# facebookresearch/FBTT-Embedding

Measured on AMD Instinct MI355X. Metric: fwd+bwd GFLOPS (true algorithmic: 3 x fwd FLOP / time), TT-EmbeddingBag E=11M D=64 ranks=[32, 32] nnz=10240, higher is better.
Workload: dtype f32

## Files before the change

### fbtt-embedding_amd/csrc/ttx_tt.hip

```cpp
#include "ttx_tt_common.h"

namespace ttx {

#include "ttx_tt_generic.inc"

__global__ __launch_bounds__(kThreads) void pool_kernel(int Nmax, const int* __restrict__ hdr, int B, int D,
                                                       const int64_t* __restrict__ rowidx,
                                                       const int64_t* __restrict__ tableidx,
                                                       const float* __restrict__ rows,
                                                       const float* __restrict__ psw, float* __restrict__ out) {
  const int n = blockIdx.x * (kThreads / 32) + threadIdx.x / 32;
  const int l = threadIdx.x & 31;
  const int N = min(Nmax, hdr[2]);
  if (n >= N) return;
  const int64_t r = rowidx[n], tb = tableidx[n];
  if (n > 0 && rowidx[n - 1] == r && tableidx[n - 1] == tb) return;
  const unsigned long long half = (threadIdx.x & 32) ? 0xffffffff00000000ull : 0x00000000ffffffffull;
  int sl = 1;
  for (;;) {
    const int c = n + sl + l;
    const bool same = c < N && rowidx[c] == r && tableidx[c] == tb;
    unsigned long long m = (__ballot(!same) & half) >> (threadIdx.x & 32);
    if (m) { sl += __builtin_ctzll(m); break; }
    sl += 32;
// ... 961 lines not shown
    return;
  }
  constexpr int kOwnerBlock = 256;
  for (int e = tid; e < sl; e += nthreads) {
    float g = 0.f;
    for (int i0 = beg; i0 < end; i0 += kOwnerBlock) {
      const int i1 = min(end, i0 + kOwnerBlock);
      float part = 0.f;
      for (int i = i0; i < i1; ++i) part += pc[(list ? (size_t)list[i] : (size_t)i) * sl + e];
      g += part;
    }
    if (optim == TTX_OPTIM_DENSE) {
      dw[base + e] = g;
    } else {
      float sv = optim == TTX_OPTIM_ADAGRAD ? stt[base + e] : 0.f;
      wt[base + e] = apply_one(optim, g, wt[base + e], lr, eps, &sv);
      if (optim == TTX_OPTIM_ADAGRAD) stt[base + e] = sv;
    }
  }
}

#include "ttx_tt_spec.inc"

static bool spec_shape(const Dims& d) { return spec_match(d) != SPEC_NONE; }
#ifndef TTX_SUBCHUNK_NNZ
#define TTX_SUBCHUNK_NNZ 131072
#endif
#ifndef TTX_SUBCHUNKS
#define TTX_SUBCHUNKS 4
#endif
template <class S>
constexpr int mc_of(int ks) { return S::MC * (S::SUB ? ks : 1); }
static int spec_mc(const Dims& d, long long nnz) {
  const int ks = nnz >= TTX_SUBCHUNK_NNZ ? TTX_SUBCHUNKS : 1;
  switch (spec_match(d)) {
    case SPEC_32_4_32_4: return mc_of<S_32_4_32_4>(ks);
    case SPEC_16_4_16_4: return mc_of<S_16_4_16_4>(ks);
    case SPEC_32_4_32_8: return mc_of<S_32_4_32_8>(ks);
    case SPEC_16_4_16_8: return mc_of<S_16_4_16_8>(ks);
    case SPEC_64_4_64_8: return mc_of<S_64_4_64_8>(ks);
    case SPEC_64_4_64_4: return mc_of<S_64_4_64_4>(ks);
    case SPEC2_32_4_32_4: return mc_of<S2_32_4_32_4>(ks);
    case SPEC2_16_4_16_4: return mc_of<S2_16_4_16_4>(ks);
    case SPEC2_64_4_64_4: return mc_of<S2_64_4_64_4>(ks);
    case SPEC_32_8_32_8: return mc_of<S_32_8_32_8>(ks);
    case SPEC_64_8_64_8: return mc_of<S_64_8_64_8>(ks);
    case SPEC2_32_2_32_4: return mc_of<S2_32_2_32_4>(ks);
    case SPEC2_64_2_64_4: return mc_of<S2_64_2_64_4>(ks);
    case SPEC2_16_2_16_4: return mc_of<S2_16_2_16_4>(ks);
    case SPEC_16_8_16_8: return mc_of<S_16_8_16_8>(ks);
    case SPEC_128_4_128_4: return mc_of<S_128_4_128_4>(ks);
    case SPEC_128_4_128_8: return mc_of<S_128_4_128_8>(ks);
    case SPEC_128_8_128_8: return mc_of<S_128_8_128_8>(ks);
    case SPEC_32_8_32_16: return mc_of<S_32_8_32_16>(ks);
    case SPEC_32_16_32_16: return mc_of<S_32_16_32_16>(ks);
    case SPEC_16_16_16_16: return mc_of<S_16_16_16_16>(ks);
    case SPEC_64_16_64_16: return mc_of<S_64_16_64_16>(ks);
    case SPEC_32_16_32_32: return mc_of<S_32_16_32_32>(ks);
    case SPEC_16_16_16_32: return mc_of<S_16_16_16_32>(ks);
    case SPEC_32_4_32_32: return mc_of<S_32_4_32_32>(ks);
    case SPEC_16_4_16_32: return mc_of<S_16_4_16_32>(ks);
    case SPEC_32_8_32_32: return mc_of<S_32_8_32_32>(ks);
    case SPEC_16_8_16_32: return mc_of<S_16_8_16_32>(ks);
    case SPEC_16_8_16_16: return mc_of<S_16_8_16_16>(ks);
    case SPEC_64_8_64_16: return mc_of<S_64_8_64_16>(ks);
    default: return 0;
  }
// ... 804 lines not shown
  TTX_HIP(hipGetLastError());
  return TTX_OK;
}

}

using namespace ttx;

extern "C" {

#ifdef TTX_TEST_HOOKS
int ttx_debug_stamps(void* device_buffer) {
  g_stamps = (long long*)device_buffer;
  return TTX_OK;
}

int ttx_debug_skip(int32_t mask) {
  g_disable_spec = (mask & 256) ? 1 : 0;
  g_disable_pad = (mask & 32768) ? 1 : 0;
  g_no_pack = (mask >> 16) & 1;
  g_skip_launch = (mask >> 9) & 63;
  mask &= 255;
  g_debug_skip = mask;
  return TTX_OK;
}

int ttx_debug_lds_budget(int32_t bytes) {
  if (bytes < 0 || bytes > 160 * 1024) TTX_FAIL(TTX_EINVAL, "LDS budget %d out of range", bytes);
  g_lds_budget = bytes ? bytes : 160 * 1024;
  return TTX_OK;
}

int ttx_set_chunk(int32_t mc) {
  if (mc < 0 || mc > 64) TTX_FAIL(TTX_EINVAL, "chunk %d out of range 0..64", mc);
  g_chunk_override = mc;
  return TTX_OK;
}
#endif

int ttx_debug_tiles(const ttx_geom* g, int32_t* out) {
  Dims d;
  int rc = make_dims(g, &d);
  if (rc) return rc;
  if (!out) TTX_FAIL(TTX_EINVAL, "out is NULL");
  for (int i = 0; i < 6; ++i) out[i] = 0;
  if (spec_shape(d) || t4_merge_dims(d, nullptr) || t2_shape(d)) return TTX_OK;
  const TileCfg cfg = choose_tiles(d);
  if (cfg.MC <= 0) return TTX_OK;
  const Lds L = make_lds(d, cfg.MC, true, cfg.bpp, cfg.KB);
  out[0] = L.MC; out[1] = L.bpp; out[2] = L.KB; out[3] = L.ncp; out[4] = L.nkb; out[5] = L.bytes;
  return TTX_OK;
}

int ttx_debug_state(void) {
  return ((g_debug_skip | g_skip_launch | g_disable_spec | g_disable_pad | g_no_pack) ? 1 : 0) | (g_lds_budget != 160 * 1024 ? 2 : 0) |
         (g_chunk_override ? 4 : 0) | (g_stamps ? 8 : 0) | (ttx_cache_debug_state() << 4);
}

int ttx_has_test_hooks(void) {
#ifdef TTX_TEST_HOOKS
  return 1;
#else
  return 0;
#endif
}

size_t ttx_tt_forward_workspace_bytes(const ttx_geom* g, int32_t B, int32_t D, int64_t nnz) {
// ... 628 lines not shown
```

### fbtt-embedding_amd/csrc/ttx_tt_common.h

```cpp
#pragma once
#include "ttx_internal.h"

namespace ttx {

constexpr int kThreads = 256;
constexpr int kWaves = kThreads / kWave;

typedef float f32x4 __attribute__((ext_vector_type(4)));

struct CorePtrs {
  float* c[TTX_MAX_CORES];
};

struct FastDiv {
  unsigned d;
  float rcp;
};
__host__ __device__ __forceinline__ FastDiv make_fd(int d) {
  FastDiv f;
  f.d = (unsigned)(d > 0 ? d : 1);
  f.rcp = 1.0f / (float)f.d;
  return f;
}
#define make_fd_dev make_fd
// ... 2 lines not shown
    rem = n % f.d;
    return n / f.d;
  }
  unsigned q = (unsigned)((float)n * f.rcp);
  int r = (int)n - (int)(q * f.d);
  if (r < 0) { q -= 1; r += (int)f.d; }
  else if (r >= (int)f.d) { q += 1; r -= (int)f.d; }
  rem = (unsigned)r;
  return q;
}

struct Partials {
  float* pc[TTX_MAX_CORES];
  const float* psw;
  const int64_t* tableidx;
  int* hot_cnt;
  int n_hot_cnt;
  float* seg[TTX_MAX_CORES];
};

__device__ __forceinline__ void zero_hot_counters(const Partials& PC) {
  if (blockIdx.x == 0 && PC.hot_cnt)
    for (int i = threadIdx.x; i < PC.n_hot_cnt; i += blockDim.x) PC.hot_cnt[i] = 0;
}

__device__ __forceinline__ f32x4 mfma4(float a, float b, f32x4 c) {
  return __builtin_amdgcn_mfma_f32_16x16x4f32(a, b, c, 0, 0, 0);
}

__device__ __forceinline__ f32x4 mfma1(float a, float b, f32x4 c) {
  return __builtin_amdgcn_mfma_f32_4x4x1f32(a, b, c, 0, 0, 0);
}

__device__ __forceinline__ void zero_output(float* __restrict__ out, long long n) {
  if (!out) return;
  for (long long e = (long long)blockIdx.x * kThreads + threadIdx.x; e < n; e += (long long)gridDim.x * kThreads) out[e] = 0.f;
}

#ifdef TTX_TEST_HOOKS
extern int g_debug_skip;
extern int g_disable_spec;
extern long long* g_stamps;
#else
constexpr int g_debug_skip = 0;
constexpr int g_disable_spec = 0;
constexpr long long* g_stamps = nullptr;
#endif

}
```

### fbtt-embedding_amd/csrc/ttx_tt_spec.inc

```

#ifndef TTX_SETPRIO
#define TTX_SETPRIO 0
#endif
#if TTX_SETPRIO
#define TTX_PRIO(x) __builtin_amdgcn_s_setprio(x)
#else
#define TTX_PRIO(x) do {} while (0)
#endif

#ifndef TTX_WGS32
#define TTX_WGS32 2
#endif
#ifndef TTX_MFMA_TAIL
#define TTX_MFMA_TAIL 1
#endif
#ifndef TTX_BFS
#define TTX_BFS 1
#endif
#ifndef TTX_GPP
#define TTX_GPP 1
#endif
#ifndef TTX_LATEB
#define TTX_LATEB 1
#endif
// ... 92 lines not shown
template <class S, bool PAD = false>
__device__ __forceinline__ void spec_fetch_b(const float* __restrict__ B1, int pass, BBlock<S>& b, const RealDims& R) {
  const int tid = threadIdx.x;
#pragma unroll
  for (int i = 0; i < S::BV4; ++i) {
    const int e = tid + i * kThreads;
    const int row = e / (S::BW / 4), c4 = e % (S::BW / 4);
    const int col0 = S::BFS ? 0 : pass * S::PW;
    if (S::BFULL || e < S::K0 * S::BW / 4) {
      if constexpr (!PAD) {
        b.v[i] = *(const float4*)(B1 + (size_t)row * S::N1 + col0 + c4 * 4);
      } else {
        const int col = col0 + c4 * 4;
        const int bq = col / S::R2, kk = col % S::R2;
        b.v[i] = ld4_guard(B1 + (size_t)row * R.n1 + bq * R.r2 + kk, (row < R.r1 && bq < R.q1) ? R.r2 - kk : 0, B1, (R.v4 & 2) != 0);
      }
    }
  }
}
template <class S>
__device__ __forceinline__ void spec_put_b(const BBlock<S>& b, float* Bs) {
  const int tid = threadIdx.x;
#pragma unroll
  for (int i = 0; i < S::BV4; ++i) {
    const int e = tid + i * kThreads;
    const int row = e / (S::BW / 4), c4 = e % (S::BW / 4);
    if (S::BFULL || e < S::K0 * S::BW / 4) {
      float2* dst = (float2*)(Bs + row * S::LDB + c4 * 4);
      dst[0] = make_float2(b.v[i].x, b.v[i].y);
      dst[1] = make_float2(b.v[i].z, b.v[i].w);
    }
  }
}
template <class S, bool ALLA>
__device__ __forceinline__ void spec_zero_pads(float* Bs, float* Aw) {
  const int tid = threadIdx.x, lane = lane_id();
  if (S::K0P != S::K0)
    for (int e = tid; e < (S::K0P - S::K0) * S::LDB; e += kThreads) Bs[S::K0 * S::LDB + e] = 0.f;
  if (ALLA || S::K0P != S::K0)
    for (int e = lane; e < S::RG * S::szA; e += kWave) Aw[e] = 0.f;
}

template <class S, bool TRANS = false>
__device__ __forceinline__ void spec_gemm_x0(const float* Aw, const float* Bs, f32x4 (&acc)[S::PNT]) {
  const int lane = lane_id();
  const int i16 = lane & 15, kq = lane >> 4;
  const float* arow = Aw + i16 * S::LDA + 8 * kq;
  const float* bbase = Bs + 8 * kq * S::LDB + i16;
#pragma unroll
  for (int x = 0; x < S::PNT; ++x) acc[x] = (f32x4){0.f, 0.f, 0.f, 0.f};
  float bcur[S::PNT];
#pragma unroll
  for (int x = 0; x < S::PNT; ++x) bcur[x] = bbase[x * 16];
  TTX_PRIO(1);
#pragma unroll
  for (int kb = 0; kb < S::K0P; kb += 32) {
    float a[8];
#pragma unroll
    for (int t = 0; t < 8; ++t) a[t] = arow[kb + t];
    __builtin_amdgcn_sched_group_barrier(0x100, 4, 0);
#pragma unroll
    for (int t = 0; t < 8; ++t) {
      const int kn = (t < 7) ? kb + t + 1 : kb + 32;
      const float* bn = bbase + (kn < S::K0P ? kn : 0) * S::LDB;
      float bnxt[S::PNT];
#pragma unroll
// ... 206 lines not shown
        if (live) L.av[gi][i] = *(const float4*)(C.c[0] + sid0 * S::SL0 + a * S::K0 + k);
      } else {
        L.av[gi][i] = ld4_guard(C.c[0] + sid0 * R.sl0 + a * R.r1 + k, (live && a < R.q0) ? R.r1 - k : 0, C.c[0], (R.v4 & 1) != 0);
      }
    }
#pragma unroll
    for (int hr = 0; hr < S::HH * 4; ++hr) {
      const int kk = (hr / 4) * 16 + kq * 4 + hr % 4;
      if constexpr (S::FMT) {
#pragma unroll
        for (int xb = 0; xb < S::Q2 / 4; ++xb) {
          const int x = 4 * xb + t4;
          if constexpr (!PAD) L.c2[gi][hr * (S::Q2 / 4) + xb] = C.c[2][sid2 * S::SL2 + kk * S::Q2 + x];
          else L.c2[gi][hr * (S::Q2 / 4) + xb] = ld_guard(C.c[2] + sid2 * R.sl2 + kk * R.q2 + x, kk < R.r2 && x < R.q2, C.c[2]);
        }
      } else if constexpr (!PAD) {
        const float4* cg = (const float4*)(C.c[2] + sid2 * S::SL2 + kk * S::Q2);
#pragma unroll
        for (int x4 = 0; x4 < S::Q2 / 4; ++x4) {
          const float4 t = cg[x4];
          L.c2[gi][hr * S::Q2 + 4 * x4] = t.x; L.c2[gi][hr * S::Q2 + 4 * x4 + 1] = t.y;
          L.c2[gi][hr * S::Q2 + 4 * x4 + 2] = t.z; L.c2[gi][hr * S::Q2 + 4 * x4 + 3] = t.w;
        }
      } else {
        const float* cg = C.c[2] + sid2 * R.sl2 + kk * R.q2;
#pragma unroll
        for (int x4 = 0; x4 < S::Q2 / 4; ++x4) {
          const float4 t = ld4_guard(cg + 4 * x4, kk < R.r2 ? R.q2 - 4 * x4 : 0, C.c[2], (R.v4 & 4) != 0);
          L.c2[gi][hr * S::Q2 + 4 * x4] = t.x; L.c2[gi][hr * S::Q2 + 4 * x4 + 1] = t.y;
          L.c2[gi][hr * S::Q2 + 4 * x4 + 2] = t.z; L.c2[gi][hr * S::Q2 + 4 * x4 + 3] = t.w;
        }
      }
    }
  }
}

#ifndef TTX_NO_KHEAD
#define TTX_KHEAD_PARAMS const int4* k_chunk_rec, const int4* k_lrec, const int* k_lrow, const int* k_hdr, const float* k_c0, \
                         const float* k_c1, const float* k_c2,
#define TTX_KHEAD_ARGS(P, C) (P).chunk_rec, (P).lrec, (P).lrow, (P).hdr, (C).c[0], (C).c[1], (C).c[2],
#define TTX_KHEAD_ADOPT(P, C)                                                                                         \
  do {                                                                                                                \
    (P).chunk_rec = const_cast<int4*>(k_chunk_rec); (P).lrec = const_cast<int4*>(k_lrec); (P).lrow = const_cast<int*>(k_lrow); \
    (P).hdr = const_cast<int*>(k_hdr); (C).c[0] = const_cast<float*>(k_c0); (C).c[1] = const_cast<float*>(k_c1);       \
    (C).c[2] = const_cast<float*>(k_c2);                                                                              \
  } while (0)
#else
#define TTX_KHEAD_PARAMS
#define TTX_KHEAD_ARGS(P, C)
#define TTX_KHEAD_ADOPT(P, C) do { } while (0)
#endif
template <class S, bool MULTI, bool FUSE = false, bool PAD = false>
__global__ __launch_bounds__(kThreads, S::WGS) void spec_fwd_kernel(TTX_KHEAD_PARAMS Plan P, CorePtrs C, float* __restrict__ rows,
                                                             float* __restrict__ zout, long long nzero, PoolFuse F, RealDims R) {
  extern __shared__ __attribute__((aligned(16))) float smem[];
  static_assert(!FUSE || (!MULTI && !PAD), "fused pooling: single sub-chunk, exact shape");
  TTX_KHEAD_ADOPT(P, C);
  if constexpr (FUSE) zero_empty_bags(F, S::D);
  else zero_output(zout, nzero);
  const int4 cr = P.chunk_rec[blockIdx.x];
  asm volatile("" ::"s"(cr.x), "s"(cr.y), "s"(cr.z));
  const int s = cr.x, start0 = cr.y, len0 = cr.z;
  if (len0 == 0) return;
  const int lane = lane_id(), w = threadIdx.x / kWave;
  const int i16 = lane & 15, kq = lane >> 4, t4 = lane & 3;
  const __amdgpu_buffer_rsrc_t rrows = make_rsrc(rows, FUSE ? F.rows_bytes : 0u);
  float* Bs = smem + S::oB;
  float* Aw0 = smem + S::oA + w * S::RG * S::szA;
  const float* B1 = C.c[1] + (size_t)s * (PAD ? R.sl1 : S::SL1);
  const int nsub = MULTI ? (len0 + S::MC - 1) / S::MC : 1;
  const int a = i16 % S::Q0;
  FwdRecs<S> rq;
  FwdLoads<S> cur, nxt;
  BBlock<S> bb;
  if constexpr (MULTI) {
    fwd_load_recs<S>(rq, P, start0, min(S::MC, len0), w);
    fwd_load<S, PAD>(cur, rq, C, R);
    if (nsub > 1) fwd_load_recs<S>(rq, P, start0 + S::MC, min(S::MC, len0 - S::MC), w);
    spec_fetch_b<S, PAD>(B1, 0, bb, R);
    if constexpr (S::B1ONCE) {
      spec_zero_pads<S, false>(Bs, Aw0);
      spec_put_b<S>(bb, Bs);
      __syncthreads();
    }
  }
  int sc = 0;
  do {
  const int start = MULTI ? start0 + sc * S::MC : start0, len = MULTI ? min(S::MC, len0 - sc * S::MC) : len0;
  const int ngroups = (len + S::LPG - 1) / S::LPG;
  if (MULTI && sc > 0 && !S::B1ONCE) __syncthreads();
  int bstart = 0, blen = 0, bag = 0;
  if constexpr (FUSE) {
    const bool has_row = P.hdr[3] != 0;
    const WaveRecs wr = load_recs<S::GPW, S::LPG>(P, start, len, w, has_row);
    if (wr.rec.x >= 0) {
      const long long tb = F.tableidx ? F.tableidx[wr.rec.x] : (long long)(s / F.p1);
      const long long row = has_row ? (long long)wr.row : F.rowidx[wr.rec.x];
      bag = (int)(tb * F.B + row);
      const long long o0 = F.offsets[bag], o1 = F.offsets[bag + 1];
      bstart = (int)o0;
      blen = (int)(o1 - o0);
      if (wr.rec.x < o0 || wr.rec.x >= o1) blen = 0;
    }
  }
  if constexpr (!MULTI) {
    fwd_load_recs<S>(rq, P, start, len, w);
#ifndef TTX_B1_LATE
    spec_fetch_b<S, PAD>(B1, 0, bb, R);
    fwd_load<S, PAD>(cur, rq, C, R);
#else
    fwd_load<S, PAD>(cur, rq, C, R);
    spec_fetch_b<S, PAD>(B1, 0, bb, R);
#endif
  } else if (sc + 1 < nsub) {
    fwd_load<S, PAD>(nxt, rq, C, R);
    if (sc + 2 < nsub) fwd_load_recs<S>(rq, P, start0 + (sc + 2) * S::MC, min(S::MC, len0 - (sc + 2) * S::MC), w);
  }
  int4 (&rec)[S::GPW] = cur.rec;
  float4 (&av)[S::GPW][S::K0T] = cur.av;
  float (&c2)[S::GPW][FwdLoads<S>::NC2] = cur.c2;
  if (!MULTI || (sc == 0 && !S::B1ONCE)) spec_zero_pads<S, false>(Bs, Aw0);
#pragma unroll
  for (int pass = 0; pass < S::NP; ++pass) {
    if (pass > 0 && !S::B1ONCE) __syncthreads();
    if (S::B1ONCE ? (pass == 0 && !MULTI) : true) {
      spec_put_b<S>(bb, Bs);
      if (!S::B1ONCE) {
        if (pass + 1 < S::NP) spec_fetch_b<S, PAD>(B1, pass + 1, bb, R);
        else if (MULTI && sc + 1 < nsub) spec_fetch_b<S, PAD>(B1, 0, bb, R);
      }
      __syncthreads();
    }
    const float* Bp = Bs + (S::BFS ? pass * S::PW : 0);
#pragma unroll
    for (int gi = 0; gi < S::GPW; ++gi) {
      const int g = w + gi * kWaves;
      if (g >= ngroups) continue;
      float* Aw = Aw0 + (S::RG > 1 ? gi : 0) * S::szA;
      if (S::NP == 1 || pass == 0) {
#pragma unroll
        for (int i = 0; i < S::K0T; ++i) {
          float2* dst = (float2*)(Aw + i16 * S::LDA + 4 * (kq + 4 * i));
          dst[0] = make_float2(av[gi][i].x, av[gi][i].y);
          dst[1] = make_float2(av[gi][i].z, av[gi][i].w);
        }
      }
      f32x4 acc[S::PNT];
      spec_gemm_x0<S, true>(Aw, Bp, acc);
      const int nrow = rec[gi].x;
      constexpr int NVT = S::NVT, PERT = S::PERT;
      float v[NVT];
      if constexpr (S::FMT) {
#pragma unroll
        for (int bl = 0; bl < S::BPP; ++bl)
#pragma unroll
          for (int xb = 0; xb < S::Q2 / 4; ++xb) {
            f32x4 o = {0.f, 0.f, 0.f, 0.f};
#pragma unroll
            for (int h = 0; h < S::HH; ++h)
#pragma unroll
              for (int r = 0; r < 4; ++r) o = mfma1(acc[bl * S::HH + h][r], c2[gi][(h * 4 + r) * (S::Q2 / 4) + xb], o);
#pragma unroll
            for (int i = 0; i < 4; ++i) v[(i * S::BPP + bl) * (S::Q2 / 4) + xb] = o[i];
          }
      } else {
#pragma unroll
        for (int bl = 0; bl < S::BPP; ++bl)
#pragma unroll
          for (int x = 0; x < S::Q2; ++x) {
            float sacc = 0.f;
#pragma unroll
            for (int h = 0; h < S::HH; ++h)
#pragma unroll
              for (int r = 0; r < 4; ++r) sacc = fmaf(acc[bl * S::HH + h][r], c2[gi][(h * 4 + r) * S::Q2 + x], sacc);
            v[bl * S::Q2 + x] = sacc;
          }
      }
      swap32_step<NVT>(v);
      swap16_step<NVT / 2>(v);
      if constexpr (S::FMT) {
        if (nrow >= 0) {
#pragma unroll
          for (int u = 0; u < PERT; ++u) {
            const int idx = kq * PERT + u;
            const int ao = idx / (S::BPP * (S::Q2 / 4)), bl = (idx / (S::Q2 / 4)) % S::BPP, x = 4 * (idx % (S::Q2 / 4)) + t4;
            const int bq = pass * S::BPP + bl;
            if constexpr (PAD) {
              if (ao < R.q0 && bq < R.q1 && x < R.q2) rows[(size_t)nrow * R.D + (ao * R.q1 + bq) * R.q2 + x] = v[u];
            } else {
              spec_store_out<1, FUSE>(rows, rrows, (size_t)nrow * S::D + (ao * S::Q1 + bq) * S::Q2 + x, v + u);
            }
          }
        }
      } else if constexpr (PAD) {
        if (nrow >= 0 && a < R.q0) {
#pragma unroll
          for (int j = 0; j < PERT; ++j) {
            const int idx = kq * PERT + j;
            const int bq = pass * S::BPP + idx / S::Q2, x = idx % S::Q2;
            if (bq < R.q1 && x < R.q2) rows[(size_t)nrow * R.D + (a * R.q1 + bq) * R.q2 + x] = v[j];
          }
        }
      } else if (nrow >= 0) {
        spec_store_out<PERT, FUSE>(rows, rrows, (size_t)nrow * S::D + (a * S::Q1 + pass * S::BPP) * S::Q2 + kq * PERT, v);
      }
    }
  }
  if constexpr (FUSE) pool_arrive<S::D>(F, rrows, bstart, blen, bag);
  if constexpr (MULTI) cur = nxt;
  } while (MULTI && ++sc < nsub);
}

template <bool NT>
__device__ __forceinline__ void spec_st(float v, float* p) {
  if (NT) __builtin_nontemporal_store(v, p); else *p = v;
}

template <bool NT>
__device__ __forceinline__ void spec_st4(const f32x4& v, float* p) {
  if (NT) __builtin_nontemporal_store(v, (f32x4*)p); else *(f32x4*)p = v;
}

template <class S>
struct BwdLoads {
  static constexpr int NG4 = (S::LPR * S::D / 4 + 15) / 16;
  float4 av[S::GPW][S::K0T];
  float4 gv4[S::GPW][NG4];
  float gsw4[S::GPW][NG4];
  f32x4 c2q[S::GPW][S::LPR][S::HH][S::Q2 / 4];
  int4 myrec[S::GPW][S::LPR];
  int pos0[S::GPW][S::LPR], pos2[S::GPW][S::LPR];
  const float* gp[S::GPW][S::NPL];
  float gsw[S::GPW];
};
template <class S>
__device__ __forceinline__ int pick2(const int (&f)[S::LPR], int k) { return f[0] + (f[S::LPR - 1] - f[0]) * k; }
template <class S>
struct BwdRecs {
  int4 rec[S::GPW][S::LPR];
// ... 99 lines not shown
        L.gv4[gi][i].x *= sw; L.gv4[gi][i].y *= sw; L.gv4[gi][i].z *= sw; L.gv4[gi][i].w *= sw;
      } else if constexpr (UNC) {
        const long long row = (long long)pick2<S>(bagrow[gi], k);
        L.gv4[gi][i] = *(const float4*)(d_output + ((size_t)table * B + row) * S::D + rem);
        if (PC.psw) L.gsw4[gi][i] = PC.psw[n >= 0 ? n : 0];
      } else if (n >= 0 && ((S::LPR * S::D / 4) % 16 == 0 || e < S::LPR * S::D)) {
        const long long row = (long long)pick2<S>(bagrow[gi], k);
        L.gv4[gi][i] = *(const float4*)(d_output + ((size_t)table * B + row) * S::D + rem);
        if (PC.psw) {
          const float sw = PC.psw[n];
          L.gv4[gi][i].x *= sw; L.gv4[gi][i].y *= sw; L.gv4[gi][i].z *= sw; L.gv4[gi][i].w *= sw;
        }
      }
    }
#pragma unroll
    for (int k = 0; k < S::LPR; ++k)
#pragma unroll
      for (int h = 0; h < S::HH; ++h) {
        const int kk = h * 16 + i16;
        const size_t sid2 = (size_t)(L.myrec[gi][k].x >= 0 ? L.myrec[gi][k].z : 0);
        const float* cg = PAD ? C.c[2] + sid2 * R.sl2 + kk * R.q2 : C.c[2] + sid2 * S::SL2 + kk * S::Q2;
#pragma unroll
        for (int x4 = 0; x4 < S::Q2 / 4; ++x4) {
          if constexpr (!PAD) {
            L.c2q[gi][k][h][x4] = *(const f32x4*)(cg + 4 * x4);
          } else {
            const float4 t = ld4_guard(cg + 4 * x4, kk < R.r2 ? R.q2 - 4 * x4 : 0, C.c[2], (R.v4 & 4) != 0);
            L.c2q[gi][k][h][x4] = (f32x4){t.x, t.y, t.z, t.w};
          }
        }
      }
  }
}
template <class S, bool UNC = false>
__device__ __forceinline__ void bwd_put(const BwdLoads<S>& L, int gi, float* Aw, float* Gw) {
  const int lane = lane_id(), i16 = lane & 15, kq = lane >> 4;
#pragma unroll
  for (int i = 0; i < S::K0T; ++i) {
    const int e = 4 * (i16 + 16 * i);
    float2* dst = (float2*)(Aw + (kq * 4 + e / S::K0) * S::LDA + e % S::K0);
    dst[0] = make_float2(L.av[gi][i].x, L.av[gi][i].y);
    dst[1] = make_float2(L.av[gi][i].z, L.av[gi][i].w);
  }
#pragma unroll
  for (int i = 0; i < (S::GPP ? 0 : BwdLoads<S>::NG4); ++i) {
    const int e = 4 * (i16 + 16 * i);
    if ((S::LPR * S::D / 4) % 16 == 0 || e < S::LPR * S::D) {
      if constexpr (UNC) {
        const float sw = L.gsw4[gi][i];
        int nn[S::LPR];
#pragma unroll
        for (int k = 0; k < S::LPR; ++k) nn[k] = L.myrec[gi][k].x;
        const bool there = pick2<S>(nn, (e / S::D) % S::LPR) >= 0;
        *(float4*)(Gw + (kq * S::LPR + e / S::D) * S::GD + e % S::D) =
            there ? make_float4(L.gv4[gi][i].x * sw, L.gv4[gi][i].y * sw, L.gv4[gi][i].z * sw, L.gv4[gi][i].w * sw)
                  : make_float4(0.f, 0.f, 0.f, 0.f);
      } else {
        *(float4*)(Gw + (kq * S::LPR + e / S::D) * S::GD + e % S::D) = L.gv4[gi][i];
      }
    }
  }
}
template <class S>
struct GPass { float4 v[S::NPL]; };
template <class S, bool PAD>
__device__ __forceinline__ GPass<S> bwd_fetch_g(const BwdLoads<S>& L, int gi, int pass, const RealDims& R) {
  constexpr int NF = S::BPP * S::Q2;
  static_assert(NF <= 16 * S::NPL, "NPL float4s per lane of the quarter");
  const int i16 = lane_id() & 15;
  const float sw = L.gsw[gi];
  GPass<S> out;
#pragma unroll
  for (int j = 0; j < S::NPL; ++j) {
    const int f = i16 + 16 * j;
    const int rr = f % (NF / 4), bl = rr / (S::Q2 / 4), x = 4 * (rr % (S::Q2 / 4));
    float4 g = make_float4(0.f, 0.f, 0.f, 0.f);
    if (L.gp[gi][j]) {
      if constexpr (!PAD) {
        g = *(const float4*)(L.gp[gi][j] + pass * S::BPP * S::Q2);
      } else {
        g = ld4_guard(L.gp[gi][j] + pass * S::BPP * R.q2, (pass * S::BPP + bl < R.q1) ? R.q2 - x : 0, L.gp[gi][j], (R.v4 & 4) != 0);
      }
      g.x *= sw; g.y *= sw; g.z *= sw; g.w *= sw;
    }
    out.v[j] = g;
  }
  return out;
}
template <class S>
__device__ __forceinline__ void bwd_put_g(const GPass<S>& g, float* Gw) {
  constexpr int NF = S::BPP * S::Q2;
  const int lane = lane_id(), i16 = lane & 15, kq = lane >> 4;
#pragma unroll
  for (int j = 0; j < S::NPL; ++j) {
    const int f = i16 + 16 * j;
    if (f >= NF) continue;
    const int a = f / (NF / 4), rr = f % (NF / 4), bl = rr / (S::Q2 / 4), x = 4 * (rr % (S::Q2 / 4));
    *(float4*)(Gw + kq * S::GD + (a * S::BPP + bl) * S::Q2 + x) = g.v[j];
  }
}

template <class S, bool PAD, bool NT>
__device__ __forceinline__ void st_pc1(float v, float* __restrict__ pc1, int k0, int colp, const RealDims& R) {
  if constexpr (!PAD) {
    spec_st<NT>(v, pc1 + k0 * S::N1 + colp);
  } else {
    const int bq = colp / S::R2, kk = colp % S::R2;
    if (k0 < R.r1 && bq < R.q1 && kk < R.r2) spec_st<NT>(v, pc1 + (size_t)k0 * R.n1 + bq * R.r2 + kk);
  }
}

template <class S, bool MULTI, bool PAD = false>
__global__ __launch_bounds__(kThreads, (PAD && S::GPP) ? 2 : S::WGS) void spec_bwd_kernel(TTX_KHEAD_PARAMS Plan P, CorePtrs C, int B, int p1,
                                                             const int64_t* __restrict__ rowidx,
                                                             const float* __restrict__ d_output,
                                                             Partials PC, int dbg, long long* stamps, RealDims R) {
  extern __shared__ __attribute__((aligned(16))) float smem[];
  TTX_KHEAD_ADOPT(P, C);
  zero_hot_counters(PC);
  const int chunk = blockIdx.x;
#define SSTAMP(i) do { if (stamps && threadIdx.x == 0) stamps[(size_t)chunk * 16 + (i)] = wall_clock64(); } while (0)
  SSTAMP(0);
  const int4 cr = P.chunk_rec[chunk];
  const int hdr3 = P.hdr[3];
  asm volatile("" ::"v"(cr.x), "v"(cr.y), "v"(cr.z), "v"(cr.w), "v"(hdr3));
  const int s = cr.x, start0 = cr.y, len0 = cr.z;
  if (len0 == 0) return;
  SSTAMP(1);
  if (dbg & 16) { if (threadIdx.x == 0 && len0 < 0) PC.pc[0][0] = 0.f; return; }
  const int tid = threadIdx.x, lane = lane_id(), w = tid / kWave;
  const int i16 = lane & 15, kq = lane >> 4;
  float* Bs = smem + S::oB;
  float* Aw0 = smem + S::oA + w * S::RG * S::szA;
  float* Xw0 = smem + S::oX + w * S::RG * S::szX;
  float* Gw0 = smem + S::oG + w * S::RG * S::szGb;
  const int table = PC.tableidx ? (int)PC.tableidx[P.lrec[start0].x] : s / p1;
  const bool has_row = hdr3 != 0;
  const float* B1 = C.c[1] + (size_t)s * (PAD ? R.sl1 : S::SL1);
  float* pc1 = PC.pc[1] + (size_t)cr.w * (PAD ? R.sl1 : S::SL1);
  f32x4 acc2p[MULTI ? S::NP : 1][S::K0T][S::TPW];
  if (MULTI) {
#pragma unroll
    for (int pp = 0; pp < S::NP; ++pp)
#pragma unroll
      for (int y = 0; y < S::K0T; ++y)
#pragma unroll
        for (int x = 0; x < S::TPW; ++x) acc2p[pp][y][x] = (f32x4){0.f, 0.f, 0.f, 0.f};
  }

  const int nsub = MULTI ? (len0 + S::MC - 1) / S::MC : 1;
  BwdRecs<S> rq;
  BwdLoads<S> cur, nxt;
  BBlock<S> bb;
  if constexpr (MULTI) {
    bwd_load_recs<S>(rq, P, start0, min(S::MC, len0), w, has_row, rowidx);
    bwd_load<S, PAD>(cur, rq, P, C, PC, has_row, table, B, rowidx, d_output, R);
    if (nsub > 1) bwd_load_recs<S>(rq, P, start0 + S::MC, min(S::MC, len0 - S::MC), w, has_row, rowidx);
    spec_fetch_b<S, PAD>(B1, 0, bb, R);
    if constexpr (S::B1ONCE) {
      spec_zero_pads<S, true>(Bs, Aw0);
      spec_put_b<S>(bb, Bs);
      __syncthreads();
    }
  }
  int sc = 0;
  do {
  const int start = MULTI ? start0 + sc * S::MC : start0, len = MULTI ? min(S::MC, len0 - sc * S::MC) : len0;
  const int ngroups = (len + S::LPG - 1) / S::LPG;
  if (MULTI && sc > 0) __syncthreads();
  SSTAMP(10);
  if (MULTI && sc < 4) SSTAMP(11 + sc);

  if constexpr (!MULTI) {
    bwd_load_recs<S>(rq, P, start, len, w, has_row, rowidx);
#ifndef TTX_B1_LATE
    spec_fetch_b<S, PAD>(B1, 0, bb, R);
#endif
    bwd_load<S, PAD, !PAD>(cur, rq, P, C, PC, has_row, table, B, rowidx, d_output, R);
  } else {
    if (sc + 1 < nsub) {
      bwd_load<S, PAD>(nxt, rq, P, C, PC, has_row, table, B, rowidx, d_output, R);
      if (sc + 2 < nsub) bwd_load_recs<S>(rq, P, start0 + (sc + 2) * S::MC, min(S::MC, len0 - (sc + 2) * S::MC), w, has_row, rowidx);
    }
  }
  float4 (&av)[S::GPW][S::K0T] = cur.av;
  float4 (&gv4)[S::GPW][BwdLoads<S>::NG4] = cur.gv4;
#define c2(GI, K, H, X) cur.c2q[GI][K][H][(X) / 4][(X) % 4]
  int4 (&myrec)[S::GPW][S::LPR] = cur.myrec;
  SSTAMP(3);
  if (dbg & 32) { if (myrec[0][0].x == -7 && myrec[S::GPW - 1][S::LPR - 1].y == -9) PC.pc[0][0] = 1.f; return; }
#ifdef TTX_B1_LATE
  if (!MULTI) spec_fetch_b<S, PAD>(B1, 0, bb, R);
#endif
  if (!MULTI || (sc == 0 && !S::B1ONCE)) spec_zero_pads<S, true>(Bs, Aw0);
  if (S::COOP) {
#pragma unroll
    for (int gi = 0; gi < S::GPW; ++gi)
      if (w + gi * kWaves >= ngroups)
        for (int e = lane; e < S::szX; e += kWave) Xw0[gi * S::szX + e] = 0.f;
  }
  if (dbg & 64) {
    float keep = bb.v[0].x;
#pragma unroll
    for (int gi = 0; gi < S::GPW; ++gi) {
      keep += av[gi][0].x + av[gi][S::K0T - 1].w + gv4[gi][0].y + c2(gi, 0, 0, 0) + c2(gi, S::LPR - 1, S::HH - 1, S::Q2 - 1);
    }
    if (keep == 12345.678f) PC.pc[0][0] = keep;
    return;
  }

  f32x4 pc2v[S::GPW][S::LPR][S::HH][S::Q2 / 4];
  f32x4 da[S::GPW][S::K0T];
  float* scratch = smem + S::oX;
  GPass<S> gpass[S::GPP ? S::GPW : 1];

#pragma unroll
  for (int pass = 0; pass < S::NP; ++pass) {
    if (pass > 0) __syncthreads();
    if (pass == 1) SSTAMP(6);
    if (S::B1ONCE ? (pass == 0 && !MULTI) : true) {
      spec_put_b<S>(bb, Bs);
      if (!S::B1ONCE && !(TTX_LATEB && S::GPP)) {
        if (pass + 1 < S::NP) spec_fetch_b<S, PAD>(B1, pass + 1, bb, R);
        else if (MULTI && sc + 1 < nsub) spec_fetch_b<S, PAD>(B1, 0, bb, R);
      }
      __syncthreads();
    }
    const float* Bp = Bs + (S::BFS ? pass * S::PW : 0);
    if (pass == 0) SSTAMP(2);
    f32x4 acc2[S::K0T][S::TPW];
#pragma unroll
    for (int y = 0; y < S::K0T; ++y)
#pragma unroll
      for (int x = 0; x < S::TPW; ++x) acc2[y][x] = (f32x4){0.f, 0.f, 0.f, 0.f};

#pragma unroll
    for (int gi = 0; gi < S::GPW; ++gi) {
      const int g = w + gi * kWaves;
      if (g >= ngroups) continue;
      bool live[S::LPR];
#pragma unroll
      for (int k = 0; k < S::LPR; ++k) live[k] = myrec[gi][k].x >= 0;
      float* Aw = Aw0 + (S::RG > 1 ? gi : 0) * S::szA;
      float* Xw = Xw0 + (S::RG > 1 ? gi : 0) * S::szX;
      float* Gw = Gw0 + (S::RG > 1 ? gi : 0) * S::szGb;
      if (S::NP == 1 || pass == 0) {
        bwd_put<S, !MULTI && !PAD>(cur, gi, Aw, Gw);
#pragma unroll
        for (int k = 0; k < S::LPR; ++k)
#pragma unroll
          for (int h = 0; h < S::HH; ++h)
#pragma unroll
            for (int xb = 0; xb < S::Q2 / 4; ++xb) pc2v[gi][k][h][xb] = (f32x4){0.f, 0.f, 0.f, 0.f};
#pragma unroll
        for (int y = 0; y < S::K0T; ++y) da[gi][y] = (f32x4){0.f, 0.f, 0.f, 0.f};
      }
      if constexpr (S::GPP) {
        if (pass == 0) gpass[gi] = bwd_fetch_g<S, PAD>(cur, gi, 0, R);
        bwd_put_g<S>(gpass[gi], Gw);
        if (pass + 1 < S::NP) gpass[gi] = bwd_fetch_g<S, PAD>(cur, gi, pass + 1, R);
      }
      if (gi == 0 && pass == 0) SSTAMP(4);
      if (dbg & 8) continue;
      f32x4 acc[S::PNT];
      spec_gemm_x0<S>(Aw, Bp, acc);
      {
        if constexpr (S::MT) {
          const int t4 = lane & 3;
          const float* gl = Gw + kq * S::GD;
#pragma unroll
          for (int bl = 0; bl < S::BPP; ++bl) {
#pragma unroll
            for (int a = 0; a < 4; ++a)
#pragma unroll
              for (int xb = 0; xb < S::Q2 / 4; ++xb) {
                const float gB = gl[(S::GPP ? a * S::BPP + bl : a * S::Q1 + pass * S::BPP + bl) * S::Q2 + xb * 4 + t4];
#pragma unroll
                for (int h = 0; h < S::HH; ++h) pc2v[gi][0][h][xb] = mfma1(gB, acc[bl * S::HH + h][a], pc2v[gi][0][h][xb]);
              }
            float gA[S::Q2];
#pragma unroll
            for (int x4 = 0; x4 < S::Q2 / 4; ++x4) {
              const float4 t = *(const float4*)(gl + (S::GPP ? t4 * S::BPP + bl : t4 * S::Q1 + pass * S::BPP + bl) * S::Q2 + 4 * x4);
              gA[4 * x4] = t.x; gA[4 * x4 + 1] = t.y; gA[4 * x4 + 2] = t.z; gA[4 * x4 + 3] = t.w;
            }
#pragma unroll
            for (int h = 0; h < S::HH; ++h) {
              f32x4 dx = {0.f, 0.f, 0.f, 0.f};
#pragma unroll
              for (int x = 0; x < S::Q2; ++x) dx = mfma1(gA[x], c2(gi, 0, h, x), dx);
              acc[bl * S::HH + h] = dx;
            }
          }
        } else {
#pragma unroll
        for (int a = 0; a < 4; ++a) {
          const float* gl = Gw + (kq * S::LPR + a / S::Q0) * S::GD;
#pragma unroll
          for (int bl = 0; bl < S::BPP; ++bl) {
            float gv[S::Q2];
#pragma unroll
            for (int x = 0; x < S::Q2; ++x) gv[x] = gl[((a % S::Q0) * S::Q1 + pass * S::BPP + bl) * S::Q2 + x];
#pragma unroll
            for (int h = 0; h < S::HH; ++h) {
              const float xv = acc[bl * S::HH + h][a];
              float dx = 0.f;
#pragma unroll
              for (int x = 0; x < S::Q2; ++x) {
                pc2v[gi][a / S::Q0][h][x / 4][x % 4] = fmaf(xv, gv[x], pc2v[gi][a / S::Q0][h][x / 4][x % 4]);
                dx = fmaf(gv[x], c2(gi, a / S::Q0, h, x), dx);
              }
              acc[bl * S::HH + h][a] = dx;
            }
          }
        }
        }
        if (pass == S::NP - 1 && !(dbg & 1)) {
#pragma unroll
          for (int k = 0; k < S::LPR; ++k)
            if (live[k]) {
#pragma unroll
              for (int h = 0; h < S::HH; ++h) {
                const int kk = h * 16 + i16;
                float* o = PAD ? PC.pc[2] + (size_t)cur.pos2[gi][k] * R.sl2 + kk * R.q2
                               : PC.pc[2] + (size_t)cur.pos2[gi][k] * S::SL2 + kk * S::Q2;
                if constexpr (!PAD) {
#pragma unroll
                  for (int x = 0; x < S::Q2; ++x) spec_st<S::NT>(pc2v[gi][k][h][x / 4][x % 4], o + x);
                } else if (R.v4 & 4) {
#pragma unroll
                  for (int x4 = 0; x4 < S::Q2 / 4; ++x4)
                    if (kk < R.r2 && 4 * x4 < R.q2) spec_st4<S::NT>(pc2v[gi][k][h][x4], o + 4 * x4);
                } else {
#pragma unroll
                  for (int x = 0; x < S::Q2; ++x)
                    if (kk < R.r2 && x < R.q2) o[x] = pc2v[gi][k][h][x / 4][x % 4];
                }
              }
            }
        }
      }
      spec_store_x<S>(acc, Xw);
      if (gi == 0 && pass == 0) SSTAMP(7);
      if (dbg & 2) continue;
      TTX_PRIO(1);
      if constexpr (!S::COOP) {
        const int rbase = 8 * (kq & 1) + 4 * (kq >> 1);
#pragma unroll
        for (int t = 0; t < 4; ++t) {
          const int row = rbase + t;
          float avv[S::K0T], bv[S::PNT];
#pragma unroll
          for (int y = 0; y < S::K0T; ++y) avv[y] = Aw[row * S::LDA + y * 16 + i16];
#pragma unroll
          for (int x = 0; x < S::PNT; ++x) bv[x] = Xw[row * S::LD + x * 16 + i16];
#pragma unroll
          for (int y = 0; y < S::K0T; ++y)
#pragma unroll
            for (int x = 0; x < S::PNT; ++x) acc2[y][x] = mfma4(avv[y], bv[x], acc2[y][x]);
        }
      }
// ... 22 lines not shown
#pragma unroll
            for (int y = 0; y < S::K0T; ++y) da[gi][y] = mfma4(ac[u], bc[u][y], da[gi][y]);
#pragma unroll
          for (int u = 0; u < 4; ++u) {
            ac[u] = an[u];
#pragma unroll
            for (int y = 0; y < S::K0T; ++y) bc[u][y] = bn[u][y];
          }
          __builtin_amdgcn_sched_group_barrier(0x100, 2 + 2 * S::K0T, 0);
          __builtin_amdgcn_sched_group_barrier(0x008, 4 * S::K0T, 0);
        }
        TTX_PRIO(0);
        if (gi == 0 && pass == 0) SSTAMP(5);
        if (pass == S::NP - 1 && !(dbg & 1)) {
#pragma unroll
          for (int r = 0; r < 4; ++r)
            if (live[r / S::Q0]) {
              if constexpr (!PAD) {
                float* o = PC.pc[0] + (size_t)cur.pos0[gi][r / S::Q0] * S::SL0 + i16;
#pragma unroll
                for (int y = 0; y < S::K0T; ++y) spec_st<S::NT>(da[gi][y][r], o + (r % S::Q0) * S::K0 + y * 16);
              } else if (r % S::Q0 < R.q0) {
                float* o = PC.pc[0] + (size_t)cur.pos0[gi][r / S::Q0] * R.sl0 + (r % S::Q0) * R.r1;
#pragma unroll
                for (int y = 0; y < S::K0T; ++y)
                  if (y * 16 + i16 < R.r1) spec_st<S::NT>(da[gi][y][r], o + y * 16 + i16);
              }
            }
        }
      }
    }

    if (pass == S::NP - 1) SSTAMP(8);
    if constexpr (TTX_LATEB && S::GPP && !S::B1ONCE) {
      if (pass + 1 < S::NP) spec_fetch_b<S, PAD>(B1, pass + 1, bb, R);
    }
    if (dbg & 4) continue;
    if constexpr (S::COOP) {
      __syncthreads();
      const int rbase = 8 * (kq & 1) + 4 * (kq >> 1);
#pragma unroll
      for (int ws = 0; ws < kWaves * S::RG; ++ws) {
        const float* As = smem + S::oA + ws * S::szA;
        const float* Xs = smem + S::oX + ws * S::szX;
#pragma unroll
        for (int t = 0; t < 4; ++t) {
          const int row = rbase + t;
          float avv[S::K0T], bv[S::TPW];
#pragma unroll
          for (int y = 0; y < S::K0T; ++y) avv[y] = As[row * S::LDA + y * 16 + i16];
#pragma unroll
          for (int x = 0; x < S::TPW; ++x) bv[x] = Xs[row * S::LD + (w * S::TPW + x) * 16 + i16];
#pragma unroll
          for (int y = 0; y < S::K0T; ++y)
#pragma unroll
            for (int x = 0; x < S::TPW; ++x) acc2[y][x] = mfma4(avv[y], bv[x], acc2[y][x]);
        }
      }
      if constexpr (MULTI) {
#pragma unroll
        for (int y = 0; y < S::K0T; ++y)
#pragma unroll
          for (int x = 0; x < S::TPW; ++x) acc2p[pass][y][x] += acc2[y][x];
      } else if (!(dbg & 128)) {
#pragma unroll
        for (int y = 0; y < S::K0T; ++y)
#pragma unroll
          for (int x = 0; x < S::TPW; ++x)
#pragma unroll
            for (int rr = 0; rr < 4; ++rr)
              st_pc1<S, PAD, S::NT>(acc2[y][x][rr], pc1, y * 16 + kq * 4 + rr, pass * S::PW + (w * S::TPW + x) * 16 + i16, R);
      }
      continue;
    }
#pragma unroll
    for (int y = 0; y < S::K0T; ++y) {
      __syncthreads();
#pragma unroll
      for (int x = 0; x < S::PNT; ++x)
#pragma unroll
        for (int r = 0; r < 4; ++r) scratch[((w * S::PNT + x) * 4 + r) * 64 + lane] = acc2[y][x][r];
      __syncthreads();
      for (int e = tid; e < S::PNT * 256; e += kThreads) {
        float v = 0.f;
#pragma unroll
        for (int ww = 0; ww < kWaves; ++ww) v += scratch[ww * S::PNT * 256 + e];
        const int x = e / 256, r = (e / 64) % 4, ln = e % 64;
        st_pc1<S, PAD, S::NT>(v, pc1, y * 16 + (ln >> 4) * 4 + r, pass * S::PW + x * 16 + (ln & 15), R);
      }
    }
// ... 260 lines not shown
```

Before: 27810.

## Force prefetched register loads to land at chosen points and defer forward stores

Adds empty inline-asm 'arrive' barriers that make the compiler wait on prefetched global loads (records, A/B/C fragments, gradients) at chosen points. This controls where s_waitcnt lands, so load latency overlaps compute instead of stalling early. In the multi-chunk forward path, output stores are buffered in registers and issued after the next chunk's loads arrive. It also moves the gradient scaling into the put step, widens the pc2 stores to float4, and adds a chunk-override value of -1 that forces subchunking. These changes raise register pressure and may reorder memory waits suboptimally.

```diff
diff --git a/fbtt-embedding_amd/csrc/ttx_tt.hip b/fbtt-embedding_amd/csrc/ttx_tt.hip
--- a/fbtt-embedding_amd/csrc/ttx_tt.hip
+++ b/fbtt-embedding_amd/csrc/ttx_tt.hip
@@ -1017,7 +1017,7 @@
 template <class S>
 constexpr int mc_of(int ks) { return S::MC * (S::SUB ? ks : 1); }
 static int spec_mc(const Dims& d, long long nnz) {
-  const int ks = nnz >= TTX_SUBCHUNK_NNZ ? TTX_SUBCHUNKS : 1;
+  const int ks = (nnz >= TTX_SUBCHUNK_NNZ || g_chunk_override < 0) ? TTX_SUBCHUNKS : 1;
   switch (spec_match(d)) {
     case SPEC_32_4_32_4: return mc_of<S_32_4_32_4>(ks);
     case SPEC_16_4_16_4: return mc_of<S_16_4_16_4>(ks);
@@ -1888,7 +1888,7 @@
 }
 
 int ttx_set_chunk(int32_t mc) {
-  if (mc < 0 || mc > 64) TTX_FAIL(TTX_EINVAL, "chunk %d out of range 0..64", mc);
+  if (mc < -1 || mc > 64) TTX_FAIL(TTX_EINVAL, "chunk %d out of range -1..64", mc);
   g_chunk_override = mc;
   return TTX_OK;
 }
diff --git a/fbtt-embedding_amd/csrc/ttx_tt_common.h b/fbtt-embedding_amd/csrc/ttx_tt_common.h
--- a/fbtt-embedding_amd/csrc/ttx_tt_common.h
+++ b/fbtt-embedding_amd/csrc/ttx_tt_common.h
@@ -58,6 +58,12 @@
   return __builtin_amdgcn_mfma_f32_4x4x1f32(a, b, c, 0, 0, 0);
 }
 
+__device__ __forceinline__ void ttx_arrive(float v) { asm volatile("" ::"v"(v)); }
+__device__ __forceinline__ void ttx_arrive(int v) { asm volatile("" ::"v"(v)); }
+__device__ __forceinline__ void ttx_arrive(const f32x4& v) { asm volatile("" ::"v"(v)); }
+__device__ __forceinline__ void ttx_arrive(const float4& v) { asm volatile("" ::"v"(v.x), "v"(v.y), "v"(v.z), "v"(v.w)); }
+__device__ __forceinline__ void ttx_arrive(const int4& v) { asm volatile("" ::"v"(v.x)); }
+
 __device__ __forceinline__ void zero_output(float* __restrict__ out, long long n) {
   if (!out) return;
   for (long long e = (long long)blockIdx.x * kThreads + threadIdx.x; e < n; e += (long long)gridDim.x * kThreads) out[e] = 0.f;
diff --git a/fbtt-embedding_amd/csrc/ttx_tt_spec.inc b/fbtt-embedding_amd/csrc/ttx_tt_spec.inc
--- a/fbtt-embedding_amd/csrc/ttx_tt_spec.inc
+++ b/fbtt-embedding_amd/csrc/ttx_tt_spec.inc
@@ -148,6 +148,11 @@
     }
   }
 }
+template <class S>
+__device__ __forceinline__ void spec_arrive_b(const BBlock<S>& b) {
+#pragma unroll
+  for (int i = 0; i < S::BV4; ++i) ttx_arrive(b.v[i]);
+}
 template <class S, bool ALLA>
 __device__ __forceinline__ void spec_zero_pads(float* Bs, float* Aw) {
   const int tid = threadIdx.x, lane = lane_id();
@@ -420,6 +425,19 @@
         }
       }
     }
+  }
+}
+
+template <class S>
+__device__ __forceinline__ void fwd_arrive(const FwdLoads<S>& L, const FwdRecs<S>& Q) {
+#pragma unroll
+  for (int gi = 0; gi < S::GPW; ++gi) {
+    ttx_arrive(Q.rec[gi]);
+    ttx_arrive(L.rec[gi]);
+#pragma unroll
+    for (int i = 0; i < S::K0T; ++i) ttx_arrive(L.av[gi][i]);
+#pragma unroll
+    for (int i = 0; i < FwdLoads<S>::NC2; ++i) ttx_arrive(L.c2[gi][i]);
   }
 }
 
@@ -471,6 +489,7 @@
       spec_put_b<S>(bb, Bs);
       __syncthreads();
     }
+    fwd_arrive<S>(cur, rq);
   }
   int sc = 0;
   do {
@@ -508,6 +527,37 @@
   float4 (&av)[S::GPW][S::K0T] = cur.av;
   float (&c2)[S::GPW][FwdLoads<S>::NC2] = cur.c2;
   if (!MULTI || (sc == 0 && !S::B1ONCE)) spec_zero_pads<S, false>(Bs, Aw0);
+  auto store_rows = [&](int pass, int gi, const float* v) {
+    constexpr int PERT = S::PERT;
+    const int nrow = rec[gi].x;
+    if constexpr (S::FMT) {
+      if (nrow >= 0) {
+#pragma unroll
+        for (int u = 0; u < PERT; ++u) {
+          const int idx = kq * PERT + u;
+          const int ao = idx / (S::BPP * (S::Q2 / 4)), bl = (idx / (S::Q2 / 4)) % S::BPP, x = 4 * (idx % (S::Q2 / 4)) + t4;
+          const int bq = pass * S::BPP + bl;
+          if constexpr (PAD) {
+            if (ao < R.q0 && bq < R.q1 && x < R.q2) rows[(size_t)nrow * R.D + (ao * R.q1 + bq) * R.q2 + x] = v[u];
+          } else {
+            spec_store_out<1, FUSE>(rows, rrows, (size_t)nrow * S::D + (ao * S::Q1 + bq) * S::Q2 + x, v + u);
+          }
+        }
+      }
+    } else if constexpr (PAD) {
+      if (nrow >= 0 && a < R.q0) {
+#pragma unroll
+        for (int j = 0; j < PERT; ++j) {
+          const int idx = kq * PERT + j;
+          const int bq = pass * S::BPP + idx / S::Q2, x = idx % S::Q2;
+          if (bq < R.q1 && x < R.q2) rows[(size_t)nrow * R.D + (a * R.q1 + bq) * R.q2 + x] = v[j];
+        }
+      }
+    } else if (nrow >= 0) {
+      spec_store_out<PERT, FUSE>(rows, rrows, (size_t)nrow * S::D + (a * S::Q1 + pass * S::BPP) * S::Q2 + kq * PERT, v);
+    }
+  };
+  float vout[MULTI ? S::GPW : 1][MULTI ? S::NP : 1][S::PERT];
 #pragma unroll
   for (int pass = 0; pass < S::NP; ++pass) {
     if (pass > 0 && !S::B1ONCE) __syncthreads();
@@ -535,7 +585,6 @@
       }
       f32x4 acc[S::PNT];
       spec_gemm_x0<S, true>(Aw, Bp, acc);
-      const int nrow = rec[gi].x;
       constexpr int NVT = S::NVT, PERT = S::PERT;
       float v[NVT];
       if constexpr (S::FMT) {
@@ -566,33 +615,21 @@
       }
       swap32_step<NVT>(v);
       swap16_step<NVT / 2>(v);
-      if constexpr (S::FMT) {
-        if (nrow >= 0) {
-#pragma unroll
-          for (int u = 0; u < PERT; ++u) {
-            const int idx = kq * PERT + u;
-            const int ao = idx / (S::BPP * (S::Q2 / 4)), bl = (idx / (S::Q2 / 4)) % S::BPP, x = 4 * (idx % (S::Q2 / 4)) + t4;
-            const int bq = pass * S::BPP + bl;
-            if constexpr (PAD) {
-              if (ao < R.q0 && bq < R.q1 && x < R.q2) rows[(size_t)nrow * R.D + (ao * R.q1 + bq) * R.q2 + x] = v[u];
-            } else {
-              spec_store_out<1, FUSE>(rows, rrows, (size_t)nrow * S::D + (ao * S::Q1 + bq) * S::Q2 + x, v + u);
-            }
-          }
-        }
-      } else if constexpr (PAD) {
-        if (nrow >= 0 && a < R.q0) {
-#pragma unroll
-          for (int j = 0; j < PERT; ++j) {
-            const int idx = kq * PERT + j;
-            const int bq = pass * S::BPP + idx / S::Q2, x = idx % S::Q2;
-            if (bq < R.q1 && x < R.q2) rows[(size_t)nrow * R.D + (a * R.q1 + bq) * R.q2 + x] = v[j];
-          }
-        }
-      } else if (nrow >= 0) {
-        spec_store_out<PERT, FUSE>(rows, rrows, (size_t)nrow * S::D + (a * S::Q1 + pass * S::BPP) * S::Q2 + kq * PERT, v);
-      }
-    }
+      if constexpr (MULTI) {
+#pragma unroll
+        for (int u = 0; u < PERT; ++u) vout[gi][pass][u] = v[u];
+      } else {
+        store_rows(pass, gi, v);
+      }
+    }
+  }
+  if constexpr (MULTI) {
+    fwd_arrive<S>(nxt, rq);
+#pragma unroll
+    for (int pass = 0; pass < S::NP; ++pass)
+#pragma unroll
+      for (int gi = 0; gi < S::GPW; ++gi)
+        if (w + gi * kWaves < ngroups) store_rows(pass, gi, vout[gi][pass]);
   }
   if constexpr (FUSE) pool_arrive<S::D>(F, rrows, bstart, blen, bag);
   if constexpr (MULTI) cur = nxt;
@@ -758,6 +795,37 @@
       }
   }
 }
+template <class S>
+__device__ __forceinline__ void bwd_arrive(const BwdLoads<S>& L) {
+#pragma unroll
+  for (int gi = 0; gi < S::GPW; ++gi) {
+#pragma unroll
+    for (int i = 0; i < S::K0T; ++i) ttx_arrive(L.av[gi][i]);
+    if constexpr (!S::GPP) {
+#pragma unroll
+      for (int i = 0; i < BwdLoads<S>::NG4; ++i) { ttx_arrive(L.gv4[gi][i]); ttx_arrive(L.gsw4[gi][i]); }
+    } else {
+      ttx_arrive(L.gsw[gi]);
+    }
+#pragma unroll
+    for (int k = 0; k < S::LPR; ++k) {
+      ttx_arrive(L.myrec[gi][k]);
+      ttx_arrive(L.pos0[gi][k]);
+      ttx_arrive(L.pos2[gi][k]);
+#pragma unroll
+      for (int h = 0; h < S::HH; ++h)
+#pragma unroll
+        for (int x4 = 0; x4 < S::Q2 / 4; ++x4) ttx_arrive(L.c2q[gi][k][h][x4]);
+    }
+  }
+}
+template <class S>
+__device__ __forceinline__ void bwd_arrive_recs(const BwdRecs<S>& Q) {
+#pragma unroll
+  for (int gi = 0; gi < S::GPW; ++gi)
+#pragma unroll
+    for (int k = 0; k < S::LPR; ++k) ttx_arrive(Q.bagrow[gi][k]);
+}
 template <class S, bool UNC = false>
 __device__ __forceinline__ void bwd_put(const BwdLoads<S>& L, int gi, float* Aw, float* Gw) {
   const int lane = lane_id(), i16 = lane & 15, kq = lane >> 4;
@@ -794,7 +862,6 @@
   constexpr int NF = S::BPP * S::Q2;
   static_assert(NF <= 16 * S::NPL, "NPL float4s per lane of the quarter");
   const int i16 = lane_id() & 15;
-  const float sw = L.gsw[gi];
   GPass<S> out;
 #pragma unroll
   for (int j = 0; j < S::NPL; ++j) {
@@ -807,22 +874,23 @@
       } else {
         g = ld4_guard(L.gp[gi][j] + pass * S::BPP * R.q2, (pass * S::BPP + bl < R.q1) ? R.q2 - x : 0, L.gp[gi][j], (R.v4 & 4) != 0);
       }
-      g.x *= sw; g.y *= sw; g.z *= sw; g.w *= sw;
     }
     out.v[j] = g;
   }
   return out;
 }
 template <class S>
-__device__ __forceinline__ void bwd_put_g(const GPass<S>& g, float* Gw) {
+__device__ __forceinline__ void bwd_put_g(const BwdLoads<S>& L, int gi, const GPass<S>& g, float* Gw) {
   constexpr int NF = S::BPP * S::Q2;
   const int lane = lane_id(), i16 = lane & 15, kq = lane >> 4;
+  const float sw = L.gsw[gi];
 #pragma unroll
   for (int j = 0; j < S::NPL; ++j) {
     const int f = i16 + 16 * j;
     if (f >= NF) continue;
     const int a = f / (NF / 4), rr = f % (NF / 4), bl = rr / (S::Q2 / 4), x = 4 * (rr % (S::Q2 / 4));
-    *(float4*)(Gw + kq * S::GD + (a * S::BPP + bl) * S::Q2 + x) = g.v[j];
+    *(float4*)(Gw + kq * S::GD + (a * S::BPP + bl) * S::Q2 + x) =
+        L.gp[gi][j] ? make_float4(g.v[j].x * sw, g.v[j].y * sw, g.v[j].z * sw, g.v[j].w * sw) : make_float4(0.f, 0.f, 0.f, 0.f);
   }
 }
 
@@ -888,7 +956,32 @@
       spec_put_b<S>(bb, Bs);
       __syncthreads();
     }
-  }
+    bwd_arrive<S>(cur);
+    bwd_arrive_recs<S>(rq);
+  }
+  auto cut32 = [&]() {
+    if (!(dbg & 32)) return false;
+    if (cur.myrec[0][0].x == -7 && cur.myrec[S::GPW - 1][S::LPR - 1].y == -9) PC.pc[0][0] = 1.f;
+    return true;
+  };
+  auto cut64 = [&]() {
+    if (!(dbg & 64)) return false;
+    float keep = bb.v[0].x;
+#pragma unroll
+    for (int gi = 0; gi < S::GPW; ++gi) {
+      keep += cur.av[gi][0].x + cur.av[gi][S::K0T - 1].w + cur.gv4[gi][0].y + cur.c2q[gi][0][0][0][0] +
+              cur.c2q[gi][S::LPR - 1][S::HH - 1][(S::Q2 - 1) / 4][(S::Q2 - 1) % 4];
+    }
+    if (keep == 12345.678f) PC.pc[0][0] = keep;
+    return true;
+  };
+  if constexpr (MULTI) {
+    if (cut32() || cut64()) return;
+  }
+  auto arrive_next = [&]() {
+    bwd_arrive<S>(nxt);
+    bwd_arrive_recs<S>(rq);
+  };
   int sc = 0;
   do {
   const int start = MULTI ? start0 + sc * S::MC : start0, len = MULTI ? min(S::MC, len0 - sc * S::MC) : len0;
@@ -909,12 +1002,12 @@
       if (sc + 2 < nsub) bwd_load_recs<S>(rq, P, start0 + (sc + 2) * S::MC, min(S::MC, len0 - (sc + 2) * S::MC), w, has_row, rowidx);
     }
   }
-  float4 (&av)[S::GPW][S::K0T] = cur.av;
-  float4 (&gv4)[S::GPW][BwdLoads<S>::NG4] = cur.gv4;
 #define c2(GI, K, H, X) cur.c2q[GI][K][H][(X) / 4][(X) % 4]
   int4 (&myrec)[S::GPW][S::LPR] = cur.myrec;
   SSTAMP(3);
-  if (dbg & 32) { if (myrec[0][0].x == -7 && myrec[S::GPW - 1][S::LPR - 1].y == -9) PC.pc[0][0] = 1.f; return; }
+  if constexpr (!MULTI) {
+    if (cut32()) return;
+  }
 #ifdef TTX_B1_LATE
   if (!MULTI) spec_fetch_b<S, PAD>(B1, 0, bb, R);
 #endif
@@ -925,14 +1018,8 @@
       if (w + gi * kWaves >= ngroups)
         for (int e = lane; e < S::szX; e += kWave) Xw0[gi * S::szX + e] = 0.f;
   }
-  if (dbg & 64) {
-    float keep = bb.v[0].x;
-#pragma unroll
-    for (int gi = 0; gi < S::GPW; ++gi) {
-      keep += av[gi][0].x + av[gi][S::K0T - 1].w + gv4[gi][0].y + c2(gi, 0, 0, 0) + c2(gi, S::LPR - 1, S::HH - 1, S::Q2 - 1);
-    }
-    if (keep == 12345.678f) PC.pc[0][0] = keep;
-    return;
+  if constexpr (!MULTI) {
+    if (cut64()) return;
   }
 
   f32x4 pc2v[S::GPW][S::LPR][S::HH][S::Q2 / 4];
@@ -942,6 +1029,9 @@
 
 #pragma unroll
   for (int pass = 0; pass < S::NP; ++pass) {
+    if constexpr (MULTI && S::NP > 1) {
+      if (pass == S::NP - 1) arrive_next();
+    }
     if (pass > 0) __syncthreads();
     if (pass == 1) SSTAMP(6);
     if (S::B1ONCE ? (pass == 0 && !MULTI) : true) {
@@ -963,7 +1053,11 @@
 #pragma unroll
     for (int gi = 0; gi < S::GPW; ++gi) {
       const int g = w + gi * kWaves;
-      if (g >= ngroups) continue;
+      const bool arrive_here = MULTI && S::NP == 1 && gi == 0;
+      if (g >= ngroups) {
+        if (arrive_here) arrive_next();
+        continue;
+      }
       bool live[S::LPR];
 #pragma unroll
       for (int k = 0; k < S::LPR; ++k) live[k] = myrec[gi][k].x >= 0;
@@ -983,11 +1077,14 @@
       }
       if constexpr (S::GPP) {
         if (pass == 0) gpass[gi] = bwd_fetch_g<S, PAD>(cur, gi, 0, R);
-        bwd_put_g<S>(gpass[gi], Gw);
+        bwd_put_g<S>(cur, gi, gpass[gi], Gw);
         if (pass + 1 < S::NP) gpass[gi] = bwd_fetch_g<S, PAD>(cur, gi, pass + 1, R);
       }
       if (gi == 0 && pass == 0) SSTAMP(4);
-      if (dbg & 8) continue;
+      if (dbg & 8) {
+        if (arrive_here) arrive_next();
+        continue;
+      }
       f32x4 acc[S::PNT];
       spec_gemm_x0<S>(Aw, Bp, acc);
       {
@@ -1041,6 +1138,7 @@
           }
         }
         }
+        if (arrive_here) arrive_next();
         if (pass == S::NP - 1 && !(dbg & 1)) {
 #pragma unroll
           for (int k = 0; k < S::LPR; ++k)
@@ -1052,7 +1150,7 @@
                                : PC.pc[2] + (size_t)cur.pos2[gi][k] * S::SL2 + kk * S::Q2;
                 if constexpr (!PAD) {
 #pragma unroll
-                  for (int x = 0; x < S::Q2; ++x) spec_st<S::NT>(pc2v[gi][k][h][x / 4][x % 4], o + x);
+                  for (int x4 = 0; x4 < S::Q2 / 4; ++x4) spec_st4<S::NT>(pc2v[gi][k][h][x4], o + 4 * x4);
                 } else if (R.v4 & 4) {
 #pragma unroll
                   for (int x4 = 0; x4 < S::Q2 / 4; ++x4)
@@ -1141,30 +1239,52 @@
     }
 
     if (pass == S::NP - 1) SSTAMP(8);
+    if constexpr (!MULTI && S::NP > 1) {
+      if (pass == 0) bwd_arrive<S>(cur);
+      if constexpr (S::GPP) {
+        if (pass + 1 < S::NP) {
+#pragma unroll
+          for (int gi = 0; gi < S::GPW; ++gi)
+#pragma unroll
+            for (int j = 0; j < S::NPL; ++j) ttx_arrive(gpass[gi].v[j]);
+        }
+      }
+      if constexpr (!S::B1ONCE && !(TTX_LATEB && S::GPP)) {
+        if (pass + 1 < S::NP) spec_arrive_b<S>(bb);
+      }
+    }
     if constexpr (TTX_LATEB && S::GPP && !S::B1ONCE) {
       if (pass + 1 < S::NP) spec_fetch_b<S, PAD>(B1, pass + 1, bb, R);
     }
-    if (dbg & 4) continue;
+    constexpr bool late_b = !MULTI && TTX_LATEB && S::GPP && !S::B1ONCE && S::COOP;
+    if (!late_b && (dbg & 4)) continue;
     if constexpr (S::COOP) {
-      __syncthreads();
-      const int rbase = 8 * (kq & 1) + 4 * (kq >> 1);
-#pragma unroll
-      for (int ws = 0; ws < kWaves * S::RG; ++ws) {
-        const float* As = smem + S::oA + ws * S::szA;
-        const float* Xs = smem + S::oX + ws * S::szX;
-#pragma unroll
-        for (int t = 0; t < 4; ++t) {
-          const int row = rbase + t;
-          float avv[S::K0T], bv[S::TPW];
-#pragma unroll
-          for (int y = 0; y < S::K0T; ++y) avv[y] = As[row * S::LDA + y * 16 + i16];
-#pragma unroll
-          for (int x = 0; x < S::TPW; ++x) bv[x] = Xs[row * S::LD + (w * S::TPW + x) * 16 + i16];
-#pragma unroll
-          for (int y = 0; y < S::K0T; ++y)
-#pragma unroll
-            for (int x = 0; x < S::TPW; ++x) acc2[y][x] = mfma4(avv[y], bv[x], acc2[y][x]);
-        }
+      const bool coop_on = !late_b || !(dbg & 4);
+      if (coop_on) {
+        __syncthreads();
+        const int rbase = 8 * (kq & 1) + 4 * (kq >> 1);
+#pragma unroll
+        for (int ws = 0; ws < kWaves * S::RG; ++ws) {
+          const float* As = smem + S::oA + ws * S::szA;
+          const float* Xs = smem + S::oX + ws * S::szX;
+#pragma unroll
+          for (int t = 0; t < 4; ++t) {
+            const int row = rbase + t;
+            float avv[S::K0T], bv[S::TPW];
+#pragma unroll
+            for (int y = 0; y < S::K0T; ++y) avv[y] = As[row * S::LDA + y * 16 + i16];
+#pragma unroll
+            for (int x = 0; x < S::TPW; ++x) bv[x] = Xs[row * S::LD + (w * S::TPW + x) * 16 + i16];
+#pragma unroll
+            for (int y = 0; y < S::K0T; ++y)
+#pragma unroll
+              for (int x = 0; x < S::TPW; ++x) acc2[y][x] = mfma4(avv[y], bv[x], acc2[y][x]);
+          }
+        }
+      }
+      if constexpr (late_b) {
+        if (pass + 1 < S::NP) spec_arrive_b<S>(bb);
+        if (!coop_on) continue;
       }
       if constexpr (MULTI) {
 #pragma unroll
```

After: 27840, median of 3. About the same (+0.1%).
